# JorgeG94/metalquicha

Hardware: AMD Instinct MI355X
Metric: SCF iterations/s (whole job); MBE-2 wall time @64 fragments (higher is better)
Workload: dtype f64

## Files before the change

metalquicha_amd/csrc/kern_fock.hip:

```cpp
#include "engine.hpp"
#include <cmath>
#include <vector>
#include <cstdlib>

namespace mqc {

__device__ __forceinline__ double wave_sum(double v)
{
#pragma unroll
    for (int off = 32; off > 0; off >>= 1) v += __shfl_down(v, off, 64);
    return v;
}

template <int CTRL, int ROWMASK>
__device__ __forceinline__ double dpp_take(double v)
{
    const int lo = __builtin_amdgcn_update_dpp(0, __double2loint(v), CTRL, ROWMASK, 0xf, false);
    const int hi = __builtin_amdgcn_update_dpp(0, __double2hiint(v), CTRL, ROWMASK, 0xf, false);
    return __hiloint2double(hi, lo);
}
__device__ __forceinline__ double wave_sum_top(double v)
{
    v += dpp_take<0xB1, 0xf>(v);
    v += dpp_take<0x4E, 0xf>(v);
    v += dpp_take<0x141, 0xf>(v);
    v += dpp_take<0x140, 0xf>(v);
    v += dpp_take<0x142, 0xa>(v);
    v += dpp_take<0x143, 0xc>(v);
    return v;
}

__device__ __forceinline__ void unpack_pair(int idx, int& k, int& l)
{
    k = (int)((sqrt(8.0 * idx + 1.0) - 1.0) * 0.5);
    while ((k + 1) * (k + 2) / 2 <= idx) ++k;
    while (k * (k + 1) / 2 > idx) --k;
    l = idx - k * (k + 1) / 2;
}

__device__ __forceinline__ double readlane_f64(double x, int l)
{
    const int lo = __builtin_amdgcn_readlane(__double2loint(x), l);
    const int hi = __builtin_amdgcn_readlane(__double2hiint(x), l);
    return __hiloint2double(hi, lo);
}

template <int KCH, bool DREG, bool FULL8>
__device__ __forceinline__ void row_exchange(const double* __restrict__ rowbuf, const double* __restrict__ Di,
                                             const double* __restrict__ Dj, int n, int lane, double* acc_i, double* acc_j)
{
#pragma unroll
    for (int c = 0; c < KCH; ++c) { acc_i[c] = 0.0; acc_j[c] = 0.0; }
    constexpr int U = 8;
    int kk[KCH], tri[KCH];
#pragma unroll
    for (int c = 0; c < KCH; ++c) {
        const int k = lane + 64 * c;
        kk[c] = k < n ? k : n - 1;
        tri[c] = kk[c] * (kk[c] + 1) / 2;
    }
    for (int l0 = 0; l0 < n; l0 += U) {
        double v[U][KCH];
        const bool full = FULL8 || l0 + U <= n;
        if (full) {
            int lbase = l0 * (l0 + 1) / 2;
#pragma unroll
            for (int u = 0; u < U; ++u) {
                const int l = l0 + u;
#pragma unroll
                for (int c = 0; c < KCH; ++c) {
                    const int ia = tri[c] + l, ib = lbase + kk[c];
                    const int idx = ia > ib ? ia : ib;
                    v[u][c] = rowbuf[idx];
                }
                lbase += l + 1;
            }
        } else if constexpr (!FULL8) {
#pragma unroll
            for (int u = 0; u < U; ++u) {
                const int l = (l0 + u < n) ? l0 + u : n - 1;
                const int lbase = l * (l + 1) / 2;
#pragma unroll
                for (int c = 0; c < KCH; ++c) {
                    const int ia = tri[c] + l, ib = lbase + kk[c];
                    const int idx = ia > ib ? ia : ib;
                    v[u][c] = rowbuf[idx];
                }
            }
        }
        double dil[U], djl[U];
        if constexpr (DREG) {
            typedef double double8 __attribute__((ext_vector_type(8)));
            typedef const double8 __attribute__((address_space(4))) * scalar_ptr8;
            typedef const double __attribute__((address_space(4))) * scalar_ptr;
            if (full) {
                const double8 a = *(scalar_ptr8)(Di + l0), b = *(scalar_ptr8)(Dj + l0);
#pragma unroll
                for (int u = 0; u < U; ++u) { dil[u] = a[u]; djl[u] = b[u]; }
            } else if constexpr (!FULL8) {
#pragma unroll
                for (int u = 0; u < U; ++u) {
                    const bool live = l0 + u < n;
                    const int lr = live ? l0 + u : n - 1;
                    dil[u] = live ? ((scalar_ptr)Di)[lr] : 0.0;
                    djl[u] = live ? ((scalar_ptr)Dj)[lr] : 0.0;
                }
            }
        } else {
#pragma unroll
            for (int u = 0; u < U; ++u) {
                const bool live = l0 + u < n;
                const int lr = live ? l0 + u : n - 1;
                dil[u] = live ? Di[lr] : 0.0;
                djl[u] = live ? Dj[lr] : 0.0;
            }
        }
#pragma unroll
        for (int u = 0; u < U; ++u) {
#pragma unroll
            for (int c = 0; c < KCH; ++c) {
                acc_i[c] += v[u][c] * djl[u];
                acc_j[c] += v[u][c] * dil[u];
            }
        }
    }
}

template <int KCH, bool KLDS, int NW, int MAXU, bool DREG, bool FULL8 = false>
__global__ void __launch_bounds__(64 * NW) jk_incore_kernel(BatchView bv, int only_active)
{
    extern __shared__ double lds[];
    const int f = blockIdx.y;
    if ((only_active & 1) && bv.istate[4 * f] == ST_DONE) return;
    const int n = bv.n, np = bv.npair;
    const int tid = threadIdx.x, lane = tid & 63;
    const int wave = __builtin_amdgcn_readfirstlane(tid >> 6);
    constexpr int NTH = 64 * NW;
    const double* __restrict__ Dg = bv.D + (size_t)f * n * n;
    double* __restrict__ Jg = bv.J + (size_t)f * n * n;
    double* __restrict__ Kg = bv.K + (size_t)f * n * n;
    const double* __restrict__ M = bv.eri + (size_t)f * np * np;

    constexpr bool TUNED = FULL8 && MAXU > 0;
    constexpr int MAXU2 = (MAXU + 1) / 2;
    const int rs = TUNED ? MAXU2 * 128 : np;
    double* rowbuf = lds + (size_t)wave * rs;
    double* Dp = lds + (size_t)NW * rs;
    double* Dl = Dp + np;
    double* Kl = Dl + ((KLDS && !DREG) ? n * n : 0);

    for (int idx = tid; idx < np; idx += NTH) {
        int k, l;
        unpack_pair(idx, k, l);
        const double d = Dg[k * n + l];
        Dp[idx] = (k == l) ? d : 2.0 * d;
    }
    if (KLDS) {
        for (int idx = tid; idx < n * n; idx += NTH) { if (!DREG) Dl[idx] = Dg[idx]; Kl[idx] = 0.0; }
    }
    const double* Dsrc = (KLDS && !DREG) ? Dl : Dg;
    __syncthreads();

    const int stride = gridDim.x * NW;
    int row = blockIdx.x * NW + wave;

    if constexpr (MAXU > 0) {
        typedef double double2v __attribute__((ext_vector_type(2)));
        double v[TUNED ? 1 : MAXU];
        double2v v2[TUNED ? MAXU2 : 1], dp2[TUNED ? MAXU2 : 1];
        auto load_row = [&](int r) {
            const double* __restrict__ src = M + (size_t)r * np;
            if constexpr (TUNED) {
#pragma unroll
                for (int u = 0; u < MAXU2; ++u) {
                    const int idx = 2 * lane + 128 * u;
                    v2[u] = idx < np ? *(const double2v*)(src + idx) : (double2v){0.0, 0.0};
                }
            } else {
#pragma unroll
                for (int u = 0; u < MAXU; ++u) { const int idx = lane + 64 * u; v[u] = idx < np ? src[idx] : 0.0; }
            }
        };
        if constexpr (TUNED) {
#pragma unroll
            for (int u = 0; u < MAXU2; ++u) {
                const int idx = 2 * lane + 128 * u;
                dp2[u] = idx < np ? *(const double2v*)(Dp + idx) : (double2v){0.0, 0.0};
            }
        }
        if (row < np) load_row(row);
        while (row < np) {
            int i, j;
            unpack_pair(row, i, j);
            double accj = 0.0;
            if constexpr (TUNED) {
#pragma unroll
                for (int u = 0; u < MAXU2; ++u) {
                    *(double2v*)(rowbuf + 2 * lane + 128 * u) = v2[u];
                    accj += v2[u][0] * dp2[u][0] + v2[u][1] * dp2[u][1];
                }
            } else {
#pragma unroll
                for (int u = 0; u < MAXU; ++u) {
                    const int idx = lane + 64 * u;
                    if (idx < np) { rowbuf[idx] = v[u]; accj += v[u] * Dp[idx]; }
                }
            }
            const int nrow = row + stride;
            if (nrow < np) load_row(nrow);
            accj = wave_sum(accj);
            if (lane == 0) { Jg[i * n + j] = accj; Jg[j * n + i] = accj; }
            double acc_i[KCH], acc_j[KCH];
            if (only_active & 2) {
#pragma unroll
                for (int c = 0; c < KCH; ++c) { acc_i[c] = 0.0; acc_j[c] = 0.0; }
            } else {
                const int iu = __builtin_amdgcn_readfirstlane(i), ju = __builtin_amdgcn_readfirstlane(j);
                row_exchange<KCH, DREG, FULL8>(rowbuf, Dsrc + iu * n, Dsrc + ju * n, n, lane, acc_i, acc_j);
            }
#pragma unroll
            for (int c = 0; c < KCH; ++c) {
                const int k = lane + 64 * c;
                if (k < n) {
                    double* Kt = KLDS ? Kl : Kg;
                    atomicAdd(&Kt[i * n + k], acc_i[c]);
                    if (i != j) atomicAdd(&Kt[j * n + k], acc_j[c]);
                }
            }
            row = nrow;
        }
    } else {
        constexpr int CH = 16;
        for (; row < np; row += stride) {
            int i, j;
            unpack_pair(row, i, j);
            const double* __restrict__ src = M + (size_t)row * np;
            double accj = 0.0;
            for (int base = 0; base < np; base += 64 * CH) {
                double v[CH];
#pragma unroll
                for (int u = 0; u < CH; ++u) { const int idx = base + lane + 64 * u; v[u] = idx < np ? src[idx] : 0.0; }
#pragma unroll
                for (int u = 0; u < CH; ++u) {
                    const int idx = base + lane + 64 * u;
                    if (idx < np) { rowbuf[idx] = v[u]; accj += v[u] * Dp[idx]; }
                }
            }
            accj = wave_sum(accj);
            if (lane == 0) { Jg[i * n + j] = accj; Jg[j * n + i] = accj; }
            double acc_i[KCH], acc_j[KCH];
            row_exchange<KCH, DREG, false>(rowbuf, Dsrc + i * n, Dsrc + j * n, n, lane, acc_i, acc_j);
#pragma unroll
            for (int c = 0; c < KCH; ++c) {
                const int k = lane + 64 * c;
                if (k < n) {
                    double* Kt = KLDS ? Kl : Kg;
                    atomicAdd(&Kt[i * n + k], acc_i[c]);
                    if (i != j) atomicAdd(&Kt[j * n + k], acc_j[c]);
                }
            }
        }
    }
    if (KLDS) {
        __syncthreads();
        for (int idx = tid; idx < n * n; idx += NTH) {
            const double kv = Kl[idx];
            if (kv != 0.0) atomicAdd(&Kg[idx], kv);
        }
    }
}

constexpr int JKC_NW = 8, JKC_NT = 64 * JKC_NW;

template <int KCH, int RPT>
__global__ void __launch_bounds__(JKC_NT) jk_rowcoop_kernel(BatchView bv, int only_active)
{
    extern __shared__ double lds[];
    const int f = blockIdx.y;
    if ((only_active & 1) && bv.istate[4 * f] == ST_DONE) return;
    const int n = bv.n, np = bv.npair;
    const int tid = threadIdx.x, lane = tid & 63;
    const int wave = __builtin_amdgcn_readfirstlane(tid >> 6);
    constexpr int NPAD = RPT * JKC_NT;
    const double* __restrict__ Dg = bv.D + (size_t)f * n * n;
    double* __restrict__ Jg = bv.J + (size_t)f * n * n;
    double* __restrict__ Kg = bv.K + (size_t)f * n * n;
    const double* __restrict__ M = bv.eri + (size_t)f * np * np;
    double* rowbuf = lds;
    double* Dp = rowbuf + 2 * NPAD;
    double* Kl = Dp + NPAD;
    double* jred = Kl + (size_t)n * n;
    for (int idx = tid; idx < NPAD; idx += JKC_NT) {
        double d = 0.0;
        if (idx < np) { int k, l; unpack_pair(idx, k, l); d = Dg[k * n + l]; if (k != l) d *= 2.0; }
        Dp[idx] = d;
    }
    for (int idx = tid; idx < n * n; idx += JKC_NT) Kl[idx] = 0.0;
    __syncthreads();
    double dp[RPT];
#pragma unroll
    for (int u = 0; u < RPT; ++u) dp[u] = Dp[tid + JKC_NT * u];

    const int stride = gridDim.x;
    int row = blockIdx.x;
    double va[RPT], vb[RPT], vc[RPT];
    auto load_row = [&](int r, double* v) {
        const double* __restrict__ src = M + (size_t)r * np;
#pragma unroll
        for (int u = 0; u < RPT; ++u) { const int idx = tid + JKC_NT * u; v[u] = (r < np && idx < np) ? src[idx] : 0.0; }
    };
    load_row(row, va);
    load_row(row + stride, vb);
    load_row(row + 2 * stride, vc);
    int t = 0, prev_i = 0, prev_j = 0;
    bool have_prev = false;
    while (row < np) {
        double* buf = rowbuf + (t & 1) * NPAD;
        double accj = 0.0;
#pragma unroll
        for (int u = 0; u < RPT; ++u) { buf[tid + JKC_NT * u] = va[u]; accj += va[u] * dp[u]; }
#pragma unroll
        for (int u = 0; u < RPT; ++u) { va[u] = vb[u]; vb[u] = vc[u]; }
        load_row(row + 3 * stride, vc);
        accj = wave_sum(accj);
        if (lane == 0) jred[(t & 1) * JKC_NW + wave] = accj;
        __syncthreads();
        int i, j;
        unpack_pair(row, i, j);
        if (tid == 0) {
            double sj = 0.0;
#pragma unroll
            for (int w = 0; w < JKC_NW; ++w) sj += jred[(t & 1) * JKC_NW + w];
            Jg[i * n + j] = sj; Jg[j * n + i] = sj;
        }
        (void)have_prev; (void)prev_i; (void)prev_j;
        if (!(only_active & 2)) {
            const int iu = __builtin_amdgcn_readfirstlane(i), ju = __builtin_amdgcn_readfirstlane(j);
            const double* __restrict__ Di = Dg + (size_t)iu * n;
            const double* __restrict__ Dj = Dg + (size_t)ju * n;
            double acc_i[KCH], acc_j[KCH];
            int kk[KCH], tri[KCH];
#pragma unroll
            for (int c = 0; c < KCH; ++c) {
                acc_i[c] = 0.0; acc_j[c] = 0.0;
                const int k = lane + 64 * c;
                kk[c] = k < n ? k : n - 1;
                tri[c] = kk[c] * (kk[c] + 1) / 2;
            }
            typedef const double __attribute__((address_space(4))) * scalar_ptr;
            for (int l0 = 8 * wave; l0 < n; l0 += 8 * JKC_NW) {
#pragma unroll
                for (int u = 0; u < 8; ++u) {
                    const bool live = l0 + u < n;
                    const int l = live ? l0 + u : n - 1;
                    const int lbase = l * (l + 1) / 2;
                    const double dil = live ? ((scalar_ptr)Di)[l] : 0.0, djl = live ? ((scalar_ptr)Dj)[l] : 0.0;
#pragma unroll
                    for (int c = 0; c < KCH; ++c) {
                        const int ia = tri[c] + l, ib = lbase + kk[c];
                        const double v = buf[ia > ib ? ia : ib];
                        acc_i[c] += v * djl;
                        acc_j[c] += v * dil;
                    }
                }
            }
#pragma unroll
            for (int c = 0; c < KCH; ++c) {
                const int k = lane + 64 * c;
                if (k < n) {
                    atomicAdd(&Kl[i * n + k], acc_i[c]);
                    if (i != j) atomicAdd(&Kl[j * n + k], acc_j[c]);
                }
            }
        }
        row += stride;
        ++t;
    }
    __syncthreads();
    for (int idx = tid; idx < n * n; idx += JKC_NT) {
        const double kv = Kl[idx];
        if (kv != 0.0) atomicAdd(&Kg[idx], kv);
    }
}

__device__ __forceinline__ void row_exchange_tri(const double* __restrict__ buf, const double* __restrict__ Di,
                                                 const double* __restrict__ Dj, int i, int lane, double& acc_i, double& acc_j)
{
    typedef double double8 __attribute__((ext_vector_type(8)));
    typedef const double8 __attribute__((address_space(4))) * scalar_ptr8;
    acc_i = 0.0; acc_j = 0.0;
    const int kk = lane <= i ? lane : i;
    const int trik = kk * (kk + 1) / 2;
    typedef const double __attribute__((address_space(3))) * lds_cptr;
    const unsigned base = (unsigned)(size_t)(lds_cptr)buf;
    unsigned rowbase = base + 8u * (unsigned)trik, colbase = base + 8u * (unsigned)kk;
    asm volatile("" : "+v"(rowbase), "+v"(colbase));
    int l0 = 0, lbase = 0;
    for (; l0 + 8 <= i + 1; l0 += 8) {
        double v[8];
        const unsigned rowaddr = rowbase + 8u * (unsigned)l0;
#pragma unroll
        for (int u = 0; u < 8; ++u) {
            const int l = l0 + u;
            const unsigned coladdr = colbase + 8u * (unsigned)(lbase - u);
            const unsigned sel = rowaddr > coladdr ? rowaddr : coladdr;
            v[u] = *(lds_cptr)(size_t)(sel + 8u * (unsigned)u);
            lbase += l + 1;
        }
        const double8 a = *(scalar_ptr8)(Di + l0), b = *(scalar_ptr8)(Dj + l0);
#pragma unroll
        for (int u = 0; u < 8; ++u) {
            acc_i += v[u] * b[u];
            acc_j += v[u] * a[u];
        }
    }
    if (l0 <= i) {
        double v[8];
#pragma unroll
        for (int u = 0; u < 8; ++u) {
            const int l = __builtin_amdgcn_readfirstlane((l0 + u <= i) ? l0 + u : i);
            const int lb = __builtin_amdgcn_readfirstlane(l * (l + 1) / 2);
            const unsigned ra = rowbase + 8u * (unsigned)l, ca = colbase + 8u * (unsigned)lb;
            v[u] = *(lds_cptr)(size_t)(ra > ca ? ra : ca);
        }
        const double8 a = *(scalar_ptr8)(Di + l0), b = *(scalar_ptr8)(Dj + l0);
#pragma unroll
        for (int u = 0; u < 8; ++u) {
            const bool live = l0 + u <= i;
            acc_i += v[u] * (live ? b[u] : 0.0);
            acc_j += v[u] * (live ? a[u] : 0.0);
        }
    }
}

template <int NW, int MAXU2>
__global__ void __launch_bounds__(64 * NW) jk_tri_kernel(BatchView bv, int only_active)
{
    extern __shared__ double lds[];
    typedef double double2v __attribute__((ext_vector_type(2)));
    const int f = blockIdx.y;
    if ((only_active & 1) && bv.istate[4 * f] == ST_DONE) return;
    const int n = bv.n, np = bv.npair, pb = bv.eri_tri_pb;
    const int tid = threadIdx.x, lane = tid & 63;
    const int wave = __builtin_amdgcn_readfirstlane(tid >> 6);
    constexpr int NTH = 64 * NW;
    const double* __restrict__ Dg = bv.D + (size_t)f * n * n;
    double* __restrict__ Jg = bv.J + (size_t)f * n * n;
    double* __restrict__ Kg = bv.K + (size_t)f * n * n;
    const double* __restrict__ T = bv.eri + (size_t)f * bv.eri_stride;
    double* rowbuf = lds + (size_t)wave * pb;
    double* Dp = lds + (size_t)NW * pb;
    double* Jl = Dp + np + 2;
    double* Kl = Jl + np + 2;
    unsigned char* rz = (unsigned char*)(Kl + (size_t)n * n);
    int* ao2sh = (int*)(rz + ((np + 15) & ~15));
    double* wred = (double*)(ao2sh + 64);

    const bool screen = bv.jk_q != nullptr;
    if (screen) {
        const TopologyDev& tp = bv.topo;
        const int ns = tp.nshell;
        const double* __restrict__ Qf = bv.jk_q + (size_t)f * ns * ns;
        for (int sh = tid; sh < ns; sh += NTH) {
            const int o = tp.sh_aoff[sh], nfun = 2 * tp.sh_l[sh] + 1;
            for (int m = 0; m < nfun; ++m) ao2sh[o + m] = sh;
        }
        double qm = 0.0;
        for (int idx = tid; idx < ns * ns; idx += NTH) qm = fmax(qm, Qf[idx]);
#pragma unroll
        for (int off = 32; off > 0; off >>= 1) qm = fmax(qm, __shfl_xor(qm, off, 64));
        if (lane == 0) wred[wave] = qm;
        __syncthreads();
        double qmax = 0.0;
        for (int w = 0; w < NW; ++w) qmax = fmax(qmax, wred[w]);
        for (int idx = tid; idx < np; idx += NTH) {
            int k, l;
            unpack_pair(idx, k, l);
            rz[idx] = (Qf[ao2sh[k] * ns + ao2sh[l]] * qmax < bv.jk_qthresh) ? 1 : 0;
        }
    } else {
        for (int idx = tid; idx < np; idx += NTH) rz[idx] = 0;
    }

    for (int idx = tid; idx < np + 2; idx += NTH) {
        double d = 0.0;
        if (idx < np) {
            int k, l;
            unpack_pair(idx, k, l);
            d = Dg[k * n + l];
            if (k != l) d *= 2.0;
        }
        Dp[idx] = d;
        Jl[idx] = 0.0;
    }
    for (int idx = tid; idx < n * n; idx += NTH) Kl[idx] = 0.0;
    if (tid == 0) ao2sh[0] = 0;
    __syncthreads();

    double2v v2[MAXU2], jsc2[MAXU2];
#pragma unroll
    for (int u = 0; u < MAXU2; ++u) jsc2[u] = (double2v){0.0, 0.0};
    const int npairs = (np + 1) / 2;
    const int stride = gridDim.x * NW;
    int t = blockIdx.x * NW + wave;
    const int* __restrict__ shell_row = bv.eri_tri_sb + npairs;
    int chunks_read = 0;
    auto load_block = [&](int tt) {
        const double* __restrict__ src = T + (size_t)tt * pb;
        const int rln = np - 1 - tt;
        const bool zln = __builtin_amdgcn_readfirstlane((int)rz[rln]) != 0;
        const bool zsn = (tt < rln) ? (__builtin_amdgcn_readfirstlane((int)rz[tt]) != 0) : true;
        const int iln = __builtin_amdgcn_readfirstlane(shell_row[rln]), isn = __builtin_amdgcn_readfirstlane(shell_row[tt]);
        const int sbn = (iln + 1) * (iln + 2) / 2, sen = (tt < rln) ? sbn + (isn + 1) * (isn + 2) / 2 : sbn;
        int c0 = zln ? sbn >> 7 : 0, c1 = zsn ? (sbn + 127) >> 7 : (sen + 127) >> 7;
        if (zln && zsn) { c0 = 0; c1 = 0; }
        c0 = __builtin_amdgcn_readfirstlane(c0); c1 = __builtin_amdgcn_readfirstlane(c1);
        chunks_read += (c1 < MAXU2 ? c1 : MAXU2) - c0;
        const double* __restrict__ srcl = src + 2 * lane;
#pragma unroll
        for (int u = 0; u < MAXU2; ++u) {
            if (u >= c0 && u < c1) {
                asm volatile("" ::: "memory");
                v2[u] = (2 * lane + 128 * u < pb) ? *(const double2v*)(srcl + 128 * u) : (double2v){0.0, 0.0};
            } else {
                v2[u] = (double2v){0.0, 0.0};
            }
        }
    };
    if (t < npairs) load_block(t);
    while (t < npairs) {
        const int rl = np - 1 - t;
        const bool two = t < rl;
        const bool zl = __builtin_amdgcn_readfirstlane((int)rz[rl]) != 0;
        const bool zs = two ? (__builtin_amdgcn_readfirstlane((int)rz[t]) != 0) : true;
        const int il = __builtin_amdgcn_readfirstlane(shell_row[rl]), jl = rl - il * (il + 1) / 2;
        const int is = two ? __builtin_amdgcn_readfirstlane(shell_row[t]) : 0, js = t - is * (is + 1) / 2;
        const int sb = (il + 1) * (il + 2) / 2;
        const int se = two ? sb + (is + 1) * (is + 2) / 2 : sb;
        const double dpl = Dp[rl], dps = Dp[t];
        double accl = 0.0, accs = 0.0;
        if (!(zl && zs))
#pragma unroll
        for (int u = 0; u < MAXU2; ++u) {
            const int base = 128 * u, idx = 2 * lane + base;
            const double2v x = v2[u];
            if (base + 128 <= pb) *(double2v*)(rowbuf + idx) = x;
            else if (idx < pb) *(double2v*)(rowbuf + idx) = x;
            if (base + 128 <= sb) {
                const double2v d = *(const double2v*)(Dp + idx);
                accl += x[0] * d[0] + x[1] * d[1];
                jsc2[u] += x * dpl;
            } else if (base >= sb) {
                if (base < se) {
                    const int q = idx - sb;
                    if (idx < se) {
                        accs += x[0] * Dp[q] + x[1] * Dp[q + 1];
                        atomicAdd(&Jl[q], x[0] * dps);
                        atomicAdd(&Jl[q + 1], x[1] * dps);
                    }
                }
            } else {
#pragma unroll
                for (int e = 0; e < 2; ++e) {
                    const int p = idx + e;
                    if (p < sb) {
                        accl += x[e] * Dp[p];
                        jsc2[u][e] += x[e] * dpl;
                    } else if (p < se) {
                        accs += x[e] * Dp[p - sb];
                        atomicAdd(&Jl[p - sb], x[e] * dps);
                    }
                }
            }
        }
        const int nt = t + stride;
        if (nt < npairs) load_block(nt);
        accl = wave_sum_top(accl);
        accs = wave_sum_top(accs);
        if (lane == 63) { if (!zl) atomicAdd(&Jl[rl], accl); if (!zs) atomicAdd(&Jl[t], accs); }
        double ai, aj;
        if (!zl) {
            row_exchange_tri(rowbuf, Dg + il * n, Dg + jl * n, il, lane, ai, aj);
            if (lane <= il) {
                atomicAdd(&Kl[il * n + lane], ai);
                if (il != jl) atomicAdd(&Kl[jl * n + lane], aj);
            }
        }
        if (!zs) {
            row_exchange_tri(rowbuf + sb, Dg + is * n, Dg + js * n, is, lane, ai, aj);
            if (lane <= is) {
                atomicAdd(&Kl[is * n + lane], ai);
                if (is != js) atomicAdd(&Kl[js * n + lane], aj);
            }
        }
        t = nt;
    }
#pragma unroll
    for (int u = 0; u < MAXU2; ++u) {
        const int idx = 2 * lane + 128 * u;
        if (idx < np && jsc2[u][0] != 0.0) atomicAdd(&Jl[idx], jsc2[u][0]);
        if (idx + 1 < np && jsc2[u][1] != 0.0) atomicAdd(&Jl[idx + 1], jsc2[u][1]);
    }
    if (lane == 0 && chunks_read > 0) atomicAdd((int*)&ao2sh[0], chunks_read);
    __syncthreads();
    if (tid == 0 && bv.jk_loaded) {
        if (gridDim.x == 1) bv.jk_loaded[f] = ao2sh[0];
        else atomicAdd(&bv.jk_loaded[f], ao2sh[0]);
    }
    if (gridDim.x == 1) {
        for (int idx = tid; idx < np; idx += NTH) {
            int k, l;
            unpack_pair(idx, k, l);
            const double jv = Jl[idx];
            Jg[k * n + l] = jv;
            Jg[l * n + k] = jv;
        }
        for (int idx = tid; idx < n * n; idx += NTH) {
            const int a = idx / n, b = idx - a * n;
            Kg[idx] = Kl[idx] + Kl[b * n + a];
        }
        return;
    }
    for (int idx = tid; idx < np; idx += NTH) {
        const double jv = Jl[idx];
        if (jv == 0.0) continue;
        int k, l;
        unpack_pair(idx, k, l);
        atomicAdd(&Jg[k * n + l], jv);
        if (k != l) atomicAdd(&Jg[l * n + k], jv);
    }
    for (int idx = tid; idx < n * n; idx += NTH) {
        const double kv = Kl[idx];
        if (kv == 0.0) continue;
        const int a = idx / n, b = idx - a * n;
        atomicAdd(&Kg[idx], kv);
        atomicAdd(&Kg[b * n + a], kv);
    }
}

static int jk_grid_x(const BatchView& bv, int nw)
{
    int want = (4096 + bv.nfrag - 1) / bv.nfrag;
    int maxx = (bv.npair + nw - 1) / nw;
    if (want < 1) want = 1;
    if (want > maxx) want = maxx;
    return want;
}

template <int KCH, bool KLDS, int NW, int MAXU, bool DREG, bool FULL8 = false>
static JkRoute jk_launch(const BatchView& bv, int oa, size_t lds, hipStream_t s)
{
    auto kern = jk_incore_kernel<KCH, KLDS, NW, MAXU, DREG, FULL8>;
    (void)hipFuncSetAttribute((const void*)kern, hipFuncAttributeMaxDynamicSharedMemorySize, (int)lds);
    dim3 grid(jk_grid_x(bv, NW), bv.nfrag), block(64 * NW);
    hipLaunchKernelGGL(kern, grid, block, lds, s, bv, oa);
    return {JK_WAVE, KCH, NW, MAXU, KLDS, DREG, FULL8, (int)grid.x};
}

static bool jk_rowcoop_on()
{
    static const bool on = [] { const char* e = std::getenv("MQC_HIP_JK_ROWCOOP"); return !(e && e[0] == '0'); }();
    return on;
}

__global__ void exchange_fold_kernel(BatchView bv, double* __restrict__ K, const double* __restrict__ Klr, double exx, double exx_lr)
{
    const int f = blockIdx.y;
    if (bv.istate[4 * f] == ST_DONE) return;
    const size_t nn = (size_t)bv.n * bv.n;
    const size_t i = (size_t)blockIdx.x * blockDim.x + threadIdx.x;
    if (i >= nn) return;
    const size_t o = (size_t)f * nn + i;
    K[o] = exx * K[o] + exx_lr * Klr[o];
}

void launch_exchange_fold(const BatchView& bv, double* K, const double* Klr, double exx, double exx_lr, hipStream_t s)
{
    const size_t nn = (size_t)bv.n * bv.n;
    hipLaunchKernelGGL(exchange_fold_kernel, dim3((unsigned)((nn + 255) / 256), (unsigned)bv.nfrag), dim3(256), 0, s, bv, K, Klr, exx, exx_lr);
}

JkRoute launch_jk_incore(const BatchView& bv, bool only_active, hipStream_t s)
{
    const int n = bv.n, np = bv.npair;
    if (bv.eri_tri) {
        const size_t lds = jk_tri_lds_bytes(n, np);
        auto kern = jk_tri_kernel<JK_TRI_NW, JK_TRI_MAXU2>;
        (void)hipFuncSetAttribute((const void*)kern, hipFuncAttributeMaxDynamicSharedMemorySize, (int)lds);
        static const int gx_env = [] { const char* e = std::getenv("MQC_HIP_JK_TRI_WG"); return e ? std::atoi(e) : 0; }();
        int gx = gx_env > 0 ? gx_env : (768 + bv.nfrag - 1) / bv.nfrag;
        const int maxx = ((np + 1) / 2 + JK_TRI_NW - 1) / JK_TRI_NW;
        if (gx < 1) gx = 1;
        if (gx > maxx) gx = maxx;
        if (gx > 1 && bv.jk_loaded) (void)hipMemsetAsync(bv.jk_loaded, 0, sizeof(int) * (size_t)bv.nfrag, s);
        if (gx > 1) {
            (void)hipMemsetAsync(bv.K, 0, sizeof(double) * (size_t)bv.nfrag * n * n, s);
            (void)hipMemsetAsync(bv.J, 0, sizeof(double) * (size_t)bv.nfrag * n * n, s);
        }
        hipLaunchKernelGGL(kern, dim3(gx, bv.nfrag), dim3(64 * JK_TRI_NW), lds, s, bv, only_active ? 1 : 0);
        return {JK_TRI, 1, JK_TRI_NW, JK_TRI_MAXU2, true, true, false, gx};
    }
    (void)hipMemsetAsync(bv.K, 0, sizeof(double) * (size_t)bv.nfrag * n * n, s);
    const int kch = (n + 63) / 64;
    static const int skip_exchange = [] { const char* e = std::getenv("MQC_HIP_JK_SKIP_EXCHANGE"); return (e && e[0] == '1') ? 2 : 0; }();
    const int oa = (only_active ? 1 : 0) | skip_exchange;
    const size_t LDS_MAX = 160 * 1024 - 1024;
    const size_t lds_reg = sizeof(double) * ((size_t)5 * np + (size_t)n * n);
    const size_t lds4k = sizeof(double) * ((size_t)5 * np + 2 * (size_t)n * n);
    const size_t lds4 = sizeof(double) * ((size_t)5 * np);
    const size_t lds2 = sizeof(double) * ((size_t)3 * np);
    const size_t lds_reg12 = sizeof(double) * ((size_t)13 * np + (size_t)n * n);
    if (n <= 64 && np <= 19 * 64 && np > 5 * 64 && lds_reg12 <= LDS_MAX && bv.nfrag >= 64) {
        if (np <= 10 * 64) return jk_launch<1, true, 12, 10, true>(bv, oa, lds_reg12, s);
        else if (n % 8 == 0 && np % 2 == 0 && sizeof(double) * ((size_t)12 * 10 * 128 + np + (size_t)n * n) <= LDS_MAX)
            return jk_launch<1, true, 12, 19, true, true>(bv, oa, sizeof(double) * ((size_t)12 * 10 * 128 + np + (size_t)n * n), s);
        else return jk_launch<1, true, 12, 19, true>(bv, oa, lds_reg12, s);
    } else if (n <= 64 && lds_reg <= LDS_MAX) {
        if (np <= 5 * 64) return jk_launch<1, true, 4, 5, true>(bv, oa, lds_reg, s);
        else if (np <= 10 * 64) return jk_launch<1, true, 4, 10, true>(bv, oa, lds_reg, s);
        else if (np <= 19 * 64) return jk_launch<1, true, 4, 19, true>(bv, oa, lds_reg, s);
        else return jk_launch<1, true, 4, 0, true>(bv, oa, lds_reg, s);
    } else if (lds4k <= LDS_MAX && kch <= 2) {
        return jk_launch<2, true, 4, 0, false>(bv, oa, lds4k, s);
    } else if (kch == 2 && np <= 8 * JKC_NT && sizeof(double) * ((size_t)3 * 8 * JKC_NT + (size_t)n * n + 2 * JKC_NW) <= LDS_MAX && jk_rowcoop_on()) {
        const size_t lds = sizeof(double) * ((size_t)3 * 8 * JKC_NT + (size_t)n * n + 2 * JKC_NW);
        auto kern = jk_rowcoop_kernel<2, 8>;
        (void)hipFuncSetAttribute((const void*)kern, hipFuncAttributeMaxDynamicSharedMemorySize, (int)lds);
        int gx = (2048 + bv.nfrag - 1) / bv.nfrag;
        if (gx < 1) gx = 1;
        if (gx > np) gx = np;
        hipLaunchKernelGGL(kern, dim3(gx, bv.nfrag), dim3(JKC_NT), lds, s, bv, oa);
        return {JK_ROWCOOP, 2, JKC_NW, 8, true, false, false, gx};
    } else if (lds4 <= LDS_MAX) {
        if (kch <= 2) return jk_launch<2, false, 4, 0, false>(bv, oa, lds4, s);
        else if (kch == 3) return jk_launch<3, false, 4, 0, false>(bv, oa, lds4, s);
        else return jk_launch<4, false, 4, 0, false>(bv, oa, lds4, s);
    } else {
        if (kch <= 2) return jk_launch<2, false, 2, 0, false>(bv, oa, lds2, s);
        else if (kch == 3) return jk_launch<3, false, 2, 0, false>(bv, oa, lds2, s);
        else return jk_launch<4, false, 2, 0, false>(bv, oa, lds2, s);
    }
}

}
```

Measured before the change: 312,900.

## Rework triangular exchange to use LDS density rows, DPP broadcast FMAs, and software pipelining

The per-pair exchange contraction no longer reads density rows from global memory through scalar loads. It loads them from the packed LDS density into per-lane register groups and consumes them with v_fmac_f64_dpp row_newbcast. The LDS reads of ERI rows are issued early and interleaved with the FMAs through a fully unrolled, compile-time template chain with sched_barriers. The second pair's loads are also prefetched during the first pair's atomics. Separately, the launcher caches hipFuncSetAttribute per shape and device so it is not called on every launch. The risks are hand-written DPP inline asm, hard limits on n (static_assert, at most six groups of eight rows) and higher register pressure.

```diff
diff --git a/metalquicha_amd/csrc/kern_fock.hip b/metalquicha_amd/csrc/kern_fock.hip
--- a/metalquicha_amd/csrc/kern_fock.hip
+++ b/metalquicha_amd/csrc/kern_fock.hip
@@ -383,55 +383,90 @@
     }
 }
 
-__device__ __forceinline__ void row_exchange_tri(const double* __restrict__ buf, const double* __restrict__ Di,
-                                                 const double* __restrict__ Dj, int i, int lane, double& acc_i, double& acc_j)
-{
-    typedef double double8 __attribute__((ext_vector_type(8)));
-    typedef const double8 __attribute__((address_space(4))) * scalar_ptr8;
-    acc_i = 0.0; acc_j = 0.0;
-    const int kk = lane <= i ? lane : i;
-    const int trik = kk * (kk + 1) / 2;
-    typedef const double __attribute__((address_space(3))) * lds_cptr;
-    const unsigned base = (unsigned)(size_t)(lds_cptr)buf;
-    unsigned rowbase = base + 8u * (unsigned)trik, colbase = base + 8u * (unsigned)kk;
-    asm volatile("" : "+v"(rowbase), "+v"(colbase));
-    int l0 = 0, lbase = 0;
-    for (; l0 + 8 <= i + 1; l0 += 8) {
-        double v[8];
-        const unsigned rowaddr = rowbase + 8u * (unsigned)l0;
-#pragma unroll
-        for (int u = 0; u < 8; ++u) {
-            const int l = l0 + u;
-            const unsigned coladdr = colbase + 8u * (unsigned)(lbase - u);
-            const unsigned sel = rowaddr > coladdr ? rowaddr : coladdr;
-            v[u] = *(lds_cptr)(size_t)(sel + 8u * (unsigned)u);
-            lbase += l + 1;
-        }
-        const double8 a = *(scalar_ptr8)(Di + l0), b = *(scalar_ptr8)(Dj + l0);
-#pragma unroll
-        for (int u = 0; u < 8; ++u) {
-            acc_i += v[u] * b[u];
-            acc_j += v[u] * a[u];
-        }
-    }
-    if (l0 <= i) {
-        double v[8];
-#pragma unroll
-        for (int u = 0; u < 8; ++u) {
-            const int l = __builtin_amdgcn_readfirstlane((l0 + u <= i) ? l0 + u : i);
-            const int lb = __builtin_amdgcn_readfirstlane(l * (l + 1) / 2);
-            const unsigned ra = rowbase + 8u * (unsigned)l, ca = colbase + 8u * (unsigned)lb;
-            v[u] = *(lds_cptr)(size_t)(ra > ca ? ra : ca);
-        }
-        const double8 a = *(scalar_ptr8)(Di + l0), b = *(scalar_ptr8)(Dj + l0);
-#pragma unroll
-        for (int u = 0; u < 8; ++u) {
-            const bool live = l0 + u <= i;
-            acc_i += v[u] * (live ? b[u] : 0.0);
-            acc_j += v[u] * (live ? a[u] : 0.0);
-        }
-    }
-}
+typedef const double __attribute__((address_space(3))) * lds_cptr;
+constexpr int JK_TRI_NG = 3;
+static_assert(JK_TRI_MAXU2 * 128 < (16 * JK_TRI_NG + 8) * (16 * JK_TRI_NG + 9) / 2, "density rows of the triangular exchange: more register groups");
+
+template <int L>
+__device__ __forceinline__ void fma_bcast(double& acc, double d, double v)
+{
+    asm("v_fmac_f64_dpp %0, %1, %2 row_newbcast:%3 row_mask:0xf bank_mask:0xf" : "+v"(acc) : "v"(d), "v"(v), "n"(L));
+}
+
+__device__ __forceinline__ void load_density_row(const double* Dp, int r, int i, int lane, double (&d)[JK_TRI_NG])
+{
+    const int tr = r * (r + 1) / 2;
+#pragma unroll
+    for (int g = 0; g < JK_TRI_NG; ++g) {
+        const int c = 16 * g + (lane & 15);
+        const int cc = c < i ? c : i;
+        const int ia = tr + cc, ib = cc * (cc + 1) / 2 + r;
+        const double x = Dp[ia > ib ? ia : ib];
+        d[g] = c > i ? 0.0 : (c == r ? x : 0.5 * x);
+    }
+}
+
+template <int L>
+__device__ __forceinline__ double exchange_read_full(unsigned rowbase, unsigned colbase)
+{
+    constexpr int u = L & 7;
+    const unsigned rowaddr = rowbase + 8u * (unsigned)(L - u);
+    const unsigned coladdr = colbase + 8u * (unsigned)(L * (L + 1) / 2 - u);
+    const unsigned sel = rowaddr > coladdr ? rowaddr : coladdr;
+    return *(lds_cptr)(size_t)(sel + 8u * (unsigned)u);
+}
+template <int L>
+__device__ __forceinline__ double exchange_read_last(unsigned rowbase, unsigned colbase, unsigned lastaddr)
+{
+    const unsigned rowaddr = rowbase + 8u * (unsigned)L, coladdr = colbase + 8u * (unsigned)(L * (L + 1) / 2);
+    const unsigned sel = rowaddr > coladdr ? rowaddr : coladdr;
+    return *(lds_cptr)(size_t)(sel < lastaddr ? sel : lastaddr);
+}
+template <int L, int LAST>
+__device__ __forceinline__ void exchange_steps(unsigned rowbase, unsigned colbase, unsigned lastaddr, const double (&di)[JK_TRI_NG],
+                                               const double (&dj)[JK_TRI_NG], double (&v)[8], double& acc_i, double& acc_j)
+{
+    constexpr int G = L / 8;
+    fma_bcast<L & 15>(acc_i, dj[L / 16], v[L & 7]);
+    fma_bcast<L & 15>(acc_j, di[L / 16], v[L & 7]);
+    if constexpr (G + 1 < LAST) v[L & 7] = exchange_read_full<L + 8>(rowbase, colbase);
+    else if constexpr (G + 1 == LAST) v[L & 7] = exchange_read_last<L + 8>(rowbase, colbase, lastaddr);
+    __builtin_amdgcn_sched_barrier(0);
+    if constexpr (L + 1 < 8 * (LAST + 1)) exchange_steps<L + 1, LAST>(rowbase, colbase, lastaddr, di, dj, v, acc_i, acc_j);
+}
+
+struct TriExchange {
+    unsigned rowbase, colbase, lastaddr;
+    double v[8];
+    __device__ __forceinline__ void begin(const double* buf, int i, int lane)
+    {
+        const int kk = lane <= i ? lane : i;
+        const int trik = kk * (kk + 1) / 2;
+        const unsigned base = (unsigned)(size_t)(lds_cptr)buf;
+        rowbase = base + 8u * (unsigned)trik; colbase = base + 8u * (unsigned)kk;
+        lastaddr = colbase + 8u * (unsigned)(i * (i + 1) / 2);
+        asm volatile("" : "+v"(rowbase), "+v"(colbase));
+        v[0] = exchange_read_last<0>(rowbase, colbase, lastaddr); v[1] = exchange_read_last<1>(rowbase, colbase, lastaddr);
+        v[2] = exchange_read_last<2>(rowbase, colbase, lastaddr); v[3] = exchange_read_last<3>(rowbase, colbase, lastaddr);
+        v[4] = exchange_read_last<4>(rowbase, colbase, lastaddr); v[5] = exchange_read_last<5>(rowbase, colbase, lastaddr);
+        v[6] = exchange_read_last<6>(rowbase, colbase, lastaddr); v[7] = exchange_read_last<7>(rowbase, colbase, lastaddr);
+        __builtin_amdgcn_sched_barrier(0);
+    }
+    __device__ __forceinline__ void finish(int i, double (&di)[JK_TRI_NG], double (&dj)[JK_TRI_NG], double& acc_i, double& acc_j)
+    {
+        static_assert(JK_TRI_NG == 3, "list every density register, and every count of groups, here");
+        asm volatile("s_nop 1" : "+v"(di[0]), "+v"(di[1]), "+v"(di[2]), "+v"(dj[0]), "+v"(dj[1]), "+v"(dj[2]));
+        acc_i = 0.0; acc_j = 0.0;
+        switch (i >> 3) {
+        case 0: exchange_steps<0, 0>(rowbase, colbase, lastaddr, di, dj, v, acc_i, acc_j); break;
+        case 1: exchange_steps<0, 1>(rowbase, colbase, lastaddr, di, dj, v, acc_i, acc_j); break;
+        case 2: exchange_steps<0, 2>(rowbase, colbase, lastaddr, di, dj, v, acc_i, acc_j); break;
+        case 3: exchange_steps<0, 3>(rowbase, colbase, lastaddr, di, dj, v, acc_i, acc_j); break;
+        case 4: exchange_steps<0, 4>(rowbase, colbase, lastaddr, di, dj, v, acc_i, acc_j); break;
+        default: exchange_steps<0, 5>(rowbase, colbase, lastaddr, di, dj, v, acc_i, acc_j); break;
+        }
+    }
+};
 
 template <int NW, int MAXU2>
 __global__ void __launch_bounds__(64 * NW) jk_tri_kernel(BatchView bv, int only_active)
@@ -575,19 +610,36 @@
         }
         const int nt = t + stride;
         if (nt < npairs) load_block(nt);
+        __builtin_amdgcn_fence(__ATOMIC_ACQ_REL, "wavefront");
+        double di[JK_TRI_NG], dj[JK_TRI_NG];
+        TriExchange x;
+        if (!zl) {
+            load_density_row(Dp, il, il, lane, di);
+            load_density_row(Dp, jl, il, lane, dj);
+            x.begin(rowbuf, il, lane);
+        } else if (!zs) {
+            load_density_row(Dp, is, is, lane, di);
+            load_density_row(Dp, js, is, lane, dj);
+            x.begin(rowbuf + sb, is, lane);
+        }
         accl = wave_sum_top(accl);
         accs = wave_sum_top(accs);
         if (lane == 63) { if (!zl) atomicAdd(&Jl[rl], accl); if (!zs) atomicAdd(&Jl[t], accs); }
         double ai, aj;
         if (!zl) {
-            row_exchange_tri(rowbuf, Dg + il * n, Dg + jl * n, il, lane, ai, aj);
+            x.finish(il, di, dj, ai, aj);
             if (lane <= il) {
                 atomicAdd(&Kl[il * n + lane], ai);
                 if (il != jl) atomicAdd(&Kl[jl * n + lane], aj);
             }
+            if (!zs) {
+                load_density_row(Dp, is, is, lane, di);
+                load_density_row(Dp, js, is, lane, dj);
+                x.begin(rowbuf + sb, is, lane);
+            }
         }
         if (!zs) {
-            row_exchange_tri(rowbuf + sb, Dg + is * n, Dg + js * n, is, lane, ai, aj);
+            x.finish(is, di, dj, ai, aj);
             if (lane <= is) {
                 atomicAdd(&Kl[is * n + lane], ai);
                 if (is != js) atomicAdd(&Kl[js * n + lane], aj);
@@ -684,9 +736,17 @@
 {
     const int n = bv.n, np = bv.npair;
     if (bv.eri_tri) {
-        const size_t lds = jk_tri_lds_bytes(n, np);
         auto kern = jk_tri_kernel<JK_TRI_NW, JK_TRI_MAXU2>;
-        (void)hipFuncSetAttribute((const void*)kern, hipFuncAttributeMaxDynamicSharedMemorySize, (int)lds);
+        struct TriShape { int n, np, dev; size_t lds; };
+        static thread_local TriShape last = {0, 0, -1, 0};
+        int dev = 0;
+        (void)hipGetDevice(&dev);
+        if (last.n != n || last.np != np || last.dev != dev) {
+            const size_t bytes = jk_tri_lds_bytes(n, np);
+            (void)hipFuncSetAttribute((const void*)kern, hipFuncAttributeMaxDynamicSharedMemorySize, (int)bytes);
+            last = {n, np, dev, bytes};
+        }
+        const size_t lds = last.lds;
         static const int gx_env = [] { const char* e = std::getenv("MQC_HIP_JK_TRI_WG"); return e ? std::atoi(e) : 0; }();
         int gx = gx_env > 0 ? gx_env : (768 + bv.nfrag - 1) / bv.nfrag;
         const int maxx = ((np + 1) / 2 + JK_TRI_NW - 1) / JK_TRI_NW;
```

Measured after the change: 321,500 (median of 6 runs). 1.03x the previous value.
